# mbrzus/Cross-Modality-Minipig-Gan

Measured on AMD Instinct MI355X. Metric: T1->T2 256x256 slices/sec (G+D step), higher is better.
Workload: dtype f32

## Files before the change

### cross-modality-minipig-gan_amd/csrc/conv_geom.h

```cpp
#pragma once
#include "mpgan_common.h"
#include "norm_fold.h"

namespace mpgan {

typedef float f32x16 __attribute__((ext_vector_type(16)));

constexpr int MAX_PHASES = 27;

struct Phase {
  FastDiv fMx, fMy, fMz;
  int Mz, My, Mx;
  int oz, oy, ox;
  int nz, ny, nx;
  int kz0, ky0, kx0;
  int dz0, dy0, dx0;
};

struct BwdStats {
  const float* z;
  const float* scale;
  const float* shift;
  const float* mean;
  const float* invstd;
// ... 62 lines not shown
    bool found = false;
#pragma unroll
    for (int i = 0; i < MAX_PHASES; ++i) {
      const unsigned tp = i < p.nphase ? (unsigned)(p.tile_start[i + 1] - p.tile_start[i]) : 0u;
      const unsigned lo = (tp * (unsigned)k) >> 3, sz = ((tp * (unsigned)(k + 1)) >> 3) - lo;
      if (!found && r < sz) { ph = i; mt = (int)(lo + r); found = true; }
      if (!found) r -= sz;
    }
    b.phase = ph;
    b.mt = mt;
    b.row = p.tile_start[ph] + mt;
    return b;
  }
  b.nt = (int)(w % (unsigned)p.ntiles);
  unsigned q = w / (unsigned)p.ntiles;
  if (p.phase_outer) {
    b.mt = (int)(q % (unsigned)p.mtiles);
    q /= (unsigned)p.mtiles;
    b.phase = (int)(q % (unsigned)p.nphase);
    b.split = (int)(q / (unsigned)p.nphase);
  } else {
    b.phase = (int)(q % (unsigned)p.nphase);
    q /= (unsigned)p.nphase;
    b.mt = (int)(q % (unsigned)p.mtiles);
    b.split = (int)(q / (unsigned)p.mtiles);
  }
  b.row = b.phase * p.mtiles + b.mt;
  return b;
}
__device__ __forceinline__ BlockId conv_block_id(const GatherConv& p) {
  return decode_block(p, xcd_remap(blockIdx.x, gridDim.x));
// ... 60 lines not shown
      int lo = (g->in_dhw[d] - 1) * g->stride[d] - 2 * g->pad[d] + g->k[d];
      MPGAN_CHECK_ARG(g->out_dhw[d] >= lo && g->out_dhw[d] < lo + g->stride[d],
                      "convT: out_dhw[%d]=%d outside [%d,%d)", d, g->out_dhw[d], lo, lo + g->stride[d]);
    }
  }
  return MPGAN_OK;
}

constexpr int FORM_MIN_BLOCKS_DEFAULT = 1024;
inline void set_geom_flags(GatherConv& p, const mpgan_conv_geom* g) {
  p.mm16 = (g->flags & MPGAN_CONV_MM_BF16) ? 1 : 0;
  p.min_blocks = g->min_blocks > 0 ? g->min_blocks : FORM_MIN_BLOCKS_DEFAULT;
}

bool mm16_gather_ok(const GatherConv& p);
int launch_gather_mm16(const GatherConv& p, int bn, int wraps, int pro, int ks, long maxM, hipStream_t st);

inline void build_forward(GatherConv& p, int n, const int32_t* gath_dhw, int cg, const int32_t* prod_dhw, int cp,
                          const int32_t* k, const int32_t* s, const int32_t* pad) {
  p.N = n; p.Di = gath_dhw[0]; p.Hi = gath_dhw[1]; p.Wi = gath_dhw[2]; p.Cin = cg;
  p.Do = prod_dhw[0]; p.Ho = prod_dhw[1]; p.Wo = prod_dhw[2]; p.Cout = cp;
  p.classes = 0; p.packed = 0;
  p.Kz = k[0]; p.Ky = k[1]; p.Kx = k[2];
  for (int d = 0; d < 3; ++d) { p.ostride[d] = 1; p.istride[d] = s[d]; p.kstep[d] = 1; p.dstep[d] = 1; }
  p.nphase = 1;
  Phase& ph = p.ph[0];
  ph.Mz = prod_dhw[0]; ph.My = prod_dhw[1]; ph.Mx = prod_dhw[2];
  ph.fMx = make_fastdiv(ph.Mx); ph.fMy = make_fastdiv(ph.My); ph.fMz = make_fastdiv(ph.Mz);
  ph.oz = ph.oy = ph.ox = 0;
  ph.nz = k[0]; ph.ny = k[1]; ph.nx = k[2];
  ph.kz0 = ph.ky0 = ph.kx0 = 0;
// ... 104 lines not shown
```

### cross-modality-minipig-gan_amd/csrc/conv_igemm.hip

```cpp
#include "mpgan_common.h"
#include "conv_geom.h"
#include "lds_dma.h"
#include "conv_pipe.h"
#include <stdlib.h>
#include <algorithm>
#include <type_traits>

namespace mpgan {


struct KCursor {
  int ci, jz, jy, jx;
  int delta;
  int dz, dy, dx;
  int woff;
  bool valid;
};

template <int BN, int TM, int TN, int WN, bool SCALAR>
__global__ __launch_bounds__(256) void gather_conv_kernel(const GatherConv p) {
  extern __shared__ __attribute__((aligned(16))) float lds[];
  constexpr int STAGE = (BM + BN) * PITCH;
  constexpr int BROWS = BN / 32;

// ... 1113 lines not shown
  Pipe,
  Dma,
  Kstep,
};

struct GatherChoice {
  GForm form;
  int rc;
  const char* msg;
  int code;
  int rows;
  int arg;
  int pro;
  int bn, wraps, ks;
  bool fast, scalar;
  int cin;
  bool narrow, merge;
  PatchLaunch pl;
  int smem, ntiles, grid;
};
struct BnTile { int bn, tm, tn, wn; };
static BnTile bn_tile(int bn) { return bn == 128 ? BnTile{128, 2, 2, 2} : (bn == 64 ? BnTile{64, 1, 2, 1} : BnTile{32, 1, 1, 1}); }
static bool fuses_bwd_sums(GForm f) { return f == GForm::Mm16 || f == GForm::Pipe || f == GForm::Dma || f == GForm::Kstep; }

template <int CIN, int PRO, bool NARROW, bool MERGE>
__global__ __launch_bounds__(256) void gather_patch_kernel(const GatherConv p, const PatchLaunch pl) {
  extern __shared__ __attribute__((aligned(16))) float lds[];
  typedef float f32x4 __attribute__((ext_vector_type(4)));
  constexpr int PC = CIN + 4;
  constexpr int CQ = CIN / 4;
  constexpr int LU = CIN == 16 ? 3 : (CIN == 32 ? 6 : 12);
  constexpr int WU = CIN == 16 ? 3 : (CIN == 32 ? 9 : 8);
  const int tid = threadIdx.x;
  const int lane = tid & 63, wid = tid >> 6;
  const unsigned wblk = xcd_remap(blockIdx.x, gridDim.x);
  const int phase0 = MERGE ? 0 : (int)(wblk % (unsigned)p.nphase);
  const int nph = MERGE ? p.nphase : 1;
// ... 885 lines not shown


static int select_variant(const GatherConv& p, long maxM, bool thin1, bool thin2) {
  if (thin1) return 1;
  if (thin2) return 2;
  const long mtiles = phase_tile_rows(p, BM);
  static const int force_bn = dev_env("MPGAN_DBG_BN") ? atoi(dev_env("MPGAN_DBG_BN")) : 0;
  if (force_bn == 32 || force_bn == 64 || force_bn == 128) return force_bn;
  int bn = 32;
  if (p.Cout > 64 && mtiles * ((p.Cout + 127) / 128) >= 256) bn = 128;
  else if (p.Cout > 32 && mtiles * ((p.Cout + 63) / 64) >= 256) bn = 64;
  else if (p.Cout > 64 && mtiles * ((p.Cout + 63) / 64) >= 128) bn = 64;
  return bn;
}

template <int BN, int TM, int TN, int WN, int WRAPS, int PRO, bool FAST = false, int KS = 1>
static int launch_pipe_variant(const GatherConv& p, long maxM, hipStream_t st) {
  auto kern = gather_conv_pipe_kernel<BN, TM, TN, WN, WRAPS, PRO, FAST, KS>;
  static const int lds_pad = dev_env("MPGAN_DBG_LDS_PAD") ? atoi(dev_env("MPGAN_DBG_LDS_PAD")) : 0;
  const int smem = KS * 2 * (BM + BN) * PITCH * (int)sizeof(float) + lds_pad;
  if (const int rc = raise_lds_limit<gather_conv_pipe_kernel<BN, TM, TN, WN, WRAPS, PRO, FAST, KS>>(smem, "gather_conv_pipe"))
    return rc;
  GatherConv q = p;
  const long pairs = set_tile_grid(q, BM);
  q.ntiles = (p.Cout + BN - 1) / BN;
  q.phase_outer = (long)p.Cout * p.Cin * p.Kz * p.Ky * p.Kx * 4 > (3L << 20) ? 1 : 0;
  if (q.ksplit < 1) q.ksplit = 1;
  dim3 grid((unsigned)(pairs * q.ntiles * q.ksplit));
  hipLaunchKernelGGL(kern, grid, dim3(256 * KS), smem, st, q);
  return check_launch("gather_conv_pipe");
}

static bool fast_geometry(const GatherConv& p, int bn) {
  static const bool off = dev_env("MPGAN_DBG_NO_FAST") != nullptr;
  if (off || p.nphase != 1 || p.Cout % bn != 0 || p.Cin % 32 != 0 || p.ksplit > 1) return false;
  const Phase& ph = p.ph[0];
  if (ph.nz * ph.ny * ph.nx == 0) return false;
  const int d0[3] = {ph.dz0, ph.dy0, ph.dx0}, nj[3] = {ph.nz, ph.ny, ph.nx}, M[3] = {ph.Mz, ph.My, ph.Mx};
  const int G[3] = {p.Di, p.Hi, p.Wi};
  for (int d = 0; d < 3; ++d) {
    const int lo = p.dstep[d] > 0 ? d0[d] : d0[d] + p.dstep[d] * (nj[d] - 1);
    const int hi = p.dstep[d] > 0 ? d0[d] + p.dstep[d] * (nj[d] - 1) : d0[d];
// ... 1 lines not shown
  }
  return true;
}

static bool pipe_wants_ksplit2(const GatherConv& p, int bn, long maxM) {
  static const bool off = dev_env("MPGAN_DBG_NO_KS2") != nullptr;
  if (off || p.ksplit > 1 || p.Cin % 32 != 0) return false;
  const long blocks = phase_tile_rows(p, BM) * ((p.Cout + bn - 1) / bn);
  if (blocks > 384) return false;
  int min_nk = 1 << 30;
  for (int i = 0; i < p.nphase; ++i) {
    const int nk = p.ph[i].nz * p.ph[i].ny * p.ph[i].nx * p.Cin / BK;
    if (nk > 0 && nk < min_nk) min_nk = nk;
  }
  return min_nk >= 8 && min_nk < (1 << 30);
}

static bool dma_form_ok(const GatherConv& p, int variant, long maxM) {
  static const bool off = dev_env("MPGAN_DBG_NO_DMA") != nullptr;
  if (off || p.pro.scale || p.ksplit > 1 || p.Cin % 32 != 0 || (variant != 128 && variant != 64 && variant != 32)) return false;
  if (p.stats_acc || p.fold.acc) return false;
  const long blocks = phase_tile_rows(p, BM) * ((p.Cout + variant - 1) / variant);
  if (blocks < (p.min_blocks > 0 ? p.min_blocks : FORM_MIN_BLOCKS_DEFAULT)) return false;
  for (int i = 0; i < p.nphase; ++i) {
    const int nt = p.ph[i].nz * p.ph[i].ny * p.ph[i].nx;
    if (nt < 1 || nt > 32) return false;
  }
  const long bytes_a = (long)p.N * p.Di * p.Hi * p.Wi * p.ldi * 4, ktot4 = (long)p.Kz * p.Ky * p.Kx * p.Cin * 4;
  return bytes_a < (long)HW_OOB && (long)p.Cout * ktot4 < (long)HW_OOB && ktot4 < 0xFFFF;
}
// ... 6 lines not shown
  if (const int rc = raise_lds_limit<gather_conv_dma_kernel<BN, TM, TN, WN, NST>>(smem, "gather_conv_dma")) return rc;
  GatherConv q = p;
  const long pairs = set_tile_grid(q, BM);
  q.ntiles = (p.Cout + BN - 1) / BN;
  q.phase_outer = (long)p.Cout * p.Cin * p.Kz * p.Ky * p.Kx * 4 > (3L << 20) ? 1 : 0;
  q.ksplit = 1;
  dim3 grid((unsigned)(pairs * q.ntiles));
  hipLaunchKernelGGL(kern, grid, dim3(256), smem, st, q);
  return check_launch("gather_conv_dma");
}

template <int WRAPS, int PRO>
static int launch_pipe_bn(const GatherConv& p, const GatherChoice& c, long maxM, hipStream_t st) {
  if constexpr (WRAPS == 1 && PRO == 3) {
    if (c.fast) return launch_pipe_variant<128, 2, 2, 2, 1, 3, true>(p, maxM, st);
  }
  if constexpr (WRAPS == 1 && PRO != 3) {
    if (c.ks == 2) {
      if (c.bn == 64) return launch_pipe_variant<64, 1, 2, 1, 1, PRO, false, 2>(p, maxM, st);
      return launch_pipe_variant<32, 1, 1, 1, 1, PRO, false, 2>(p, maxM, st);
    }
  }
  if (c.bn == 128) return launch_pipe_variant<128, 2, 2, 2, WRAPS, PRO>(p, maxM, st);
  if (c.bn == 64) return launch_pipe_variant<64, 1, 2, 1, WRAPS, PRO>(p, maxM, st);
  return launch_pipe_variant<32, 1, 1, 1, WRAPS, PRO>(p, maxM, st);
}

template <int WRAPS>
static int launch_pipe_pro(const GatherConv& p, const GatherChoice& c, long maxM, hipStream_t st) {
  switch (c.pro) {
// ... 389 lines not shown
      c.narrow = p.Cout <= 16;
      c.merge = c.pl.merged != 0;
      c.form = persist ? GForm::PatchPersist : GForm::Patch;
      if (persist) {
        c.pl = pp;
        c.smem = psmem;
      }
      return c;
    }
    CHOICE_REFUSE(p.stats != nullptr, "gather_conv: fused statistics of a patch-kernel geometry need 16-byte "
                                      "aligned operands (the partial-row count differs otherwise)");
  }
  CHOICE_REFUSE(p.fold.acc != nullptr, "gather_conv: fold-on-load is served by the persistent patch kernel only");
  c.rows = (int)phase_tile_rows(p, BM);
  c.ks = 1;
  const bool vec = (p.Cin % 4 == 0) && (p.ldi % 4 == 0) && ((reinterpret_cast<uintptr_t>(p.in) & 15) == 0) &&
                   ((reinterpret_cast<uintptr_t>(p.wp) & 15) == 0) &&
                   (!p.pro.scale || (((reinterpret_cast<uintptr_t>(p.pro.scale) |
                                       reinterpret_cast<uintptr_t>(p.pro.shift)) & 15) == 0 &&
                                     p.pro.n_stride % 4 == 0));
  static const bool no_pipe = dev_env("MPGAN_DBG_NO_PIPE") != nullptr;
  const bool small = (long)p.N * p.Di * p.Hi * p.Wi * p.ldi * 4 < (1L << 32) &&
                     (long)p.Cout * p.Cin * p.Kz * p.Ky * p.Kx * 4 < (1L << 32) &&
                     (long)p.N * (p.pro.n_stride > 0 ? p.pro.n_stride : 0) * 4 < (1L << 31);
  const bool mm16 = p.mm16 && vec && small && mm16_gather_ok(p);
  if (vec && small && (p.Cin % 32 == 0 || p.Cin == 16) && (!no_pipe || mm16)) {
    c.form = GForm::Pipe;
    c.wraps = p.Cin % 32 == 0 ? 1 : 2;
    if (!p.pro.scale) c.pro = 0;
    else if (p.pro.n_stride == 0 && p.pro.act == MPGAN_ACT_LEAKY && !p.pro.slope_ptr && p.pro.slope >= 0.f && p.pro.slope <= 1.f)
      c.pro = 3;
    else c.pro = p.pro.n_stride == 0 ? 1 : 2;
    const bool ks2 = c.wraps == 1 && variant != 128 && pipe_wants_ksplit2(p, variant, maxM);
    if (c.wraps == 1 && c.pro == 3 && variant == 128 && fast_geometry(p, 128)) {
      c.fast = true;
      c.code = 1128;
    } else if (c.wraps == 1 && c.pro != 3 && ks2) {
      c.ks = 2;
      c.code = 2000 + variant;
    } else if (c.wraps == 1 && c.pro == 0 && dma_form_ok(p, variant, maxM)) {
      c.form = GForm::Dma;
      c.code = 3000 + variant;
    }
    if (mm16) {
      c.form = GForm::Mm16;
      c.pro = p.pro.scale != nullptr;
      c.ks = ks2 ? 2 : 1;
      c.fast = false;
    }
    return c;
  }
  c.form = GForm::Kstep;
  c.scalar = !vec;
  return c;
}
#undef CHOICE_REFUSE

static int launch_chosen(const GatherConv& p, const GatherChoice& c, long maxM, hipStream_t st) {
  if (c.rc != MPGAN_OK) {
    set_error("%s", c.msg);
    return c.rc;
  }
// ... 83 lines not shown
    case GForm::Patch3d:
      if (c.arg) return c.pro ? launch_patch3d_instance<true, true>(p, st) : launch_patch3d_instance<false, true>(p, st);
      return c.pro ? launch_patch3d_instance<true, false>(p, st) : launch_patch3d_instance<false, false>(p, st);
    case GForm::Patch: return launch_patch<false>(p, c, c.pl, st);
    case GForm::PatchPersist: {
      static void* zp = nullptr;
      if (!zp && hipGetSymbolAddress(&zp, HIP_SYMBOL(g_patch_zero_page)) != hipSuccess) {
        zp = nullptr;
        set_error("gather_patch_persist: no address for the zero page");
        return MPGAN_ERR_HIP;
      }
      PatchLaunch pl = c.pl;
      pl.zero_page = zp;
      return launch_patch<true>(p, c, pl, st);
    }
    case GForm::Mm16: return launch_gather_mm16(p, c.bn, c.wraps, c.pro, c.ks, maxM, st);
    case GForm::Pipe: return c.wraps == 1 ? launch_pipe_pro<1>(p, c, maxM, st) : launch_pipe_pro<2>(p, c, maxM, st);
    case GForm::Dma:
      if (c.bn == 128) return launch_dma_variant<128, 2, 2, 2>(p, maxM, st);
      if (c.bn == 64) return launch_dma_variant<64, 1, 2, 1>(p, maxM, st);
      return launch_dma_variant<32, 1, 1, 1, 2>(p, maxM, st);
    case GForm::Kstep:
      if (c.scalar) {
        if (c.bn == 128) return launch_variant<128, 2, 2, 2, true>(p, maxM, st);
        if (c.bn == 64) return launch_variant<64, 1, 2, 1, true>(p, maxM, st);
        return launch_variant<32, 1, 1, 1, true>(p, maxM, st);
      }
      if (c.bn == 128) return launch_variant<128, 2, 2, 2, false>(p, maxM, st);
      if (c.bn == 64) return launch_variant<64, 1, 2, 1, false>(p, maxM, st);
      return launch_variant<32, 1, 1, 1, false>(p, maxM, st);
  }
  return MPGAN_ERR_UNSUPPORTED;
}

static int gather_kernel_name(const GatherChoice& c, char* buf, int len) {
  const char* b[2] = {"false", "true"};
  const BnTile t = bn_tile(c.bn);
  switch (c.form) {
    case GForm::ThinBf16OutRows: return snprintf(buf, len, "thin_cin1_rows_kernel<%d, true>", c.arg);
    case GForm::Cin1Rows: return snprintf(buf, len, "thin_cin1_rows_kernel<%d, false>", c.arg);
    case GForm::ThinBf16OutFull: return snprintf(buf, len, "thin_cin1_full_kernel<%d, true>", c.arg);
    case GForm::Cin1Full: return snprintf(buf, len, "thin_cin1_full_kernel<%d, false>", c.arg);
    case GForm::ThinBf16InMfma: return snprintf(buf, len, "thin_cout1_mfma_bf16_kernel");
    case GForm::ThinBf16In: return snprintf(buf, len, "thin_cout1_kernel<%d, true>", c.arg);
    case GForm::C1C1Rows4: return snprintf(buf, len, "thin_c1c1_rows4_kernel<%s>", b[c.arg]);
    case GForm::Cin1: return snprintf(buf, len, "thin_cin1_kernel<%d>", c.arg);
    case GForm::ConvtQuad: return snprintf(buf, len, "convt_quad_cout1_kernel<%d>", c.arg);
    case GForm::ConvtOct: return snprintf(buf, len, "convt_oct_cout1_kernel<%d>", c.arg);
    case GForm::Cout1: return snprintf(buf, len, "thin_cout1_kernel<%d, false>", c.arg);
    case GForm::Patch3d: return snprintf(buf, len, "gather_patch3d_c16_kernel<%s, %s>", b[c.pro], b[c.arg]);
    case GForm::Patch:
      return snprintf(buf, len, "gather_patch_kernel<%d, %d, %s, %s>", c.cin, c.pro, b[c.narrow], b[c.merge]);
// ... 338 lines not shown
```

### cross-modality-minipig-gan_amd/csrc/conv_mm16.hip

```cpp
#include "conv_pipe.h"
#include "wgrad_pipe.h"
#include <stdlib.h>

namespace mpgan {

template <int BN, int TM, int TN, int WN, int WRAPS, int PRO, int KS>
static int launch_mm16_variant(const GatherConv& p, long maxM, hipStream_t st) {
  auto kern = gather_conv_pipe_kernel<BN, TM, TN, WN, WRAPS, PRO, false, KS, true>;
  constexpr int stage_b = (BM + BN) * MM16_PITCHB;
  constexpr int loop_b = KS * 2 * stage_b;
  constexpr int fold_b = KS > 1 ? TM * TN * 16 * 256 * 4 : 0;
  constexpr int epi_b = CONV_EPI_FLOATS * 4;
  constexpr int smem = loop_b > fold_b ? (loop_b > epi_b ? loop_b : epi_b) : (fold_b > epi_b ? fold_b : epi_b);
  if (const int rc = raise_lds_limit<gather_conv_pipe_kernel<BN, TM, TN, WN, WRAPS, PRO, false, KS, true>>(
          smem, "gather_conv_pipe (bf16 operands)"))
    return rc;
  GatherConv q = p;
  const long pairs = set_tile_grid(q, BM);
  q.ntiles = (p.Cout + BN - 1) / BN;
  q.phase_outer = (long)p.Cout * p.Cin * p.Kz * p.Ky * p.Kx * 4 > (3L << 20) ? 1 : 0;
  q.ksplit = 1;
  dim3 grid((unsigned)(pairs * q.ntiles));
  hipLaunchKernelGGL(kern, grid, dim3(256 * KS), smem, st, q);
  return check_launch("gather_conv_pipe (bf16 operands)");
}

template <int WRAPS, int PRO>
static int launch_mm16_bn(const GatherConv& p, int bn, int ks, long maxM, hipStream_t st) {
  if constexpr (WRAPS == 1) {
    if (ks == 2)
      return bn == 64 ? launch_mm16_variant<64, 1, 2, 1, 1, PRO, 2>(p, maxM, st)
                      : launch_mm16_variant<32, 1, 1, 1, 1, PRO, 2>(p, maxM, st);
  }
  if (bn == 128) return launch_mm16_variant<128, 2, 2, 2, WRAPS, PRO, 1>(p, maxM, st);
  if (bn == 64) return launch_mm16_variant<64, 1, 2, 1, WRAPS, PRO, 1>(p, maxM, st);
  return launch_mm16_variant<32, 1, 1, 1, WRAPS, PRO, 1>(p, maxM, st);
}

bool mm16_gather_ok(const GatherConv& p) {
  static const bool off = dev_env("MPGAN_DBG_NO_MM16") != nullptr;
  return !off && (p.Cin % 32 == 0 || p.Cin == 16) && (!p.pro.scale || p.pro.n_stride == 0) && !p.fold.acc &&
         !p.stats_acc && p.ksplit <= 1 && !p.in_bf16 && !p.out_bf16;
}

int launch_gather_mm16(const GatherConv& p, int bn, int wraps, int pro, int ks, long maxM, hipStream_t st) {
  if (wraps == 1) return pro ? launch_mm16_bn<1, 1>(p, bn, ks, maxM, st) : launch_mm16_bn<1, 0>(p, bn, ks, maxM, st);
  return pro ? launch_mm16_bn<2, 1>(p, bn, ks, maxM, st) : launch_mm16_bn<2, 0>(p, bn, ks, maxM, st);
}

template <int BD, int BG, int TM, int TN, int WN, int PRO, bool PAD>
static int launch_wgrad_mm16_variant(const WgradParams& p, hipStream_t st) {
  auto kern = wgrad_pipe_kernel<BD, BG, TM, TN, WN, PRO, PAD, true>;
  constexpr int smem = 2 * WBK * (BD + BG) * (int)sizeof(float) + 2 * 32 * 16;
  if (const int rc = raise_lds_limit<wgrad_pipe_kernel<BD, BG, TM, TN, WN, PRO, PAD, true>>(smem, "wgrad_pipe (bf16 operands)"))
    return rc;
  dim3 grid((unsigned)p.tiles_c * p.tiles_d * p.nsplit);
  hipLaunchKernelGGL(kern, grid, dim3(256), smem, st, p);
  return check_launch("wgrad_pipe (bf16 operands)");
}

template <int PRO>
static int launch_wgrad_mm16_pad(const WgradParams& p, int BD, int BG, hipStream_t st) {
// ... 16 lines not shown
```

### cross-modality-minipig-gan_amd/csrc/conv_pipe.h

```cpp
#pragma once
#include <type_traits>
#include "mpgan_common.h"
#include "conv_geom.h"
#include "lds_dma.h"

namespace mpgan {

constexpr int BM = 128;
constexpr int BK = 32;
constexpr int PITCH = BK + 4;

#ifndef MPGAN_BWD_EPILOGUE_WALK
#define MPGAN_BWD_EPILOGUE_WALK 0
#endif

__device__ __forceinline__ void bwd_sums_add(float v, float zz, float sc, float sh, float mu, float is, bool leaky, float slope,
                                             float& b1, float& b2, float& b3) {
#pragma clang fp contract(off)
  const float y = __builtin_fmaf(zz, sc, sh);
  const float zh = (zz - mu) * is;
  const bool neg = leaky && y < 0.f;
  const float gy = neg ? v * slope : v;
  const float t3 = neg ? v * y : 0.f;
  b1 += gy;
  b2 = __builtin_fmaf(gy, zh, b2);
  b3 += t3;
}

template <int BN, int TM, int TN, int WN, bool BWC = false>
__device__ __forceinline__ void conv_epilogue(const GatherConv& p, const Phase& ph, f32x16 (&acc)[TM][TN], float* lds,
                                              long m0, int n0, long Mtot, int stats_row, bool zero_rows = false,
                                              int tid = threadIdx.x, bool active = true, const float* bias_pre = nullptr) {
  const int lane = tid & 63, wid = tid >> 6;
  const int li = lane & 31, lh = lane >> 5;
  const int wm = wid / WN, wn = wid % WN;
  const int Cout = p.Cout;
  const int ksplit_id = p.ksplit > 1 ? (int)(xcd_remap(blockIdx.x, gridDim.x) / (unsigned)(p.ntiles * p.mtiles * (p.packed ? 1 : p.nphase))) : 0;
  int* rowpix = reinterpret_cast<int*>(lds);
  const bool bw = p.bwd.part != nullptr;
  int* rowoo = rowpix + BM;
  int* rowoz = rowpix + 2 * BM;
  bool bw_vec = false;
  if constexpr (BWC) if (bw) {
    const unsigned long long npix = (unsigned long long)p.N * p.Do * p.Ho * p.Wo;
    bw_vec = !MPGAN_BWD_EPILOGUE_WALK && !p.epi.scale && !p.resid && !p.tanh_out && (Cout % 4 == 0) && (p.ldo % 4 == 0) &&
             ((reinterpret_cast<uintptr_t>(p.out) & 15) == 0) && Cout <= p.ldo && Cout <= p.bwd.ldz &&
             npix * (unsigned)p.ldo * 4ull <= 0xFFFFFFFFull && npix * (unsigned)p.bwd.ldz * 4ull <= 0xFFFFFFFFull;
  }
  if (active && tid < BM) {
    const unsigned m = (unsigned)m0 + tid;
    int pix = -1;
    if (m < (unsigned)Mtot) {
      unsigned q, umx, umy, umz;
      fdivmod(m, ph.fMx, q, umx);
      fdivmod(q, ph.fMy, q, umy);
      fdivmod(q, ph.fMz, q, umz);
      const int mx = (int)umx, my = (int)umy, mz = (int)umz;
      const int n = (int)q;
      int oz = mz * p.ostride[0] + ph.oz, oy = my * p.ostride[1] + ph.oy, ox = mx * p.ostride[2] + ph.ox;
      if (oz < p.Do && oy < p.Ho && ox < p.Wo) pix = ((n * p.Do + oz) * p.Ho + oy) * p.Wo + ox;
    }
    rowpix[tid] = pix;
    if (bw_vec) {
      const unsigned upix = pix < 0 ? 0u : (unsigned)pix;
// ... 231 lines not shown
    constexpr int WM = 4 / WN;
    float* st = lds + 1024;
    int* nvp = reinterpret_cast<int*>(lds) + 512;
    if (zero_rows && active) {
#pragma unroll
      for (int tm = 0; tm < TM; ++tm)
#pragma unroll
        for (int r = 0; r < 16; ++r) {
          const int row = (wm * TM + tm) * 32 + (r & 3) + 8 * (r >> 2) + 4 * lh;
          if (rowpix[row] < 0) {
#pragma unroll
            for (int tn = 0; tn < TN; ++tn) acc[tm][tn][r] = 0.f;
          }
        }
    }
    if (active && tid < BM) {
      const unsigned long long b = __ballot(rowpix[tid] >= 0);
      if (lane == 0) nvp[wid] = __popcll(b);
    }
#pragma unroll
    for (int tn = 0; tn < TN; ++tn) {
      const int col = (wn * TN + tn) * 32 + li;
      float sm = 0.f, sq = 0.f;
#pragma unroll
      for (int tm = 0; tm < TM; ++tm)
#pragma unroll
        for (int r = 0; r < 16; ++r) {
          const float v = acc[tm][tn][r];
          sm += v;
          sq = fmaf(v, v, sq);
        }
      sm += __shfl_xor(sm, 32, 64);
      sq += __shfl_xor(sq, 32, 64);
      if (active && lh == 0) {
        st[(wm * 2 + 0) * BN + col] = sm;
        st[(wm * 2 + 1) * BN + col] = sq;
      }
    }
    __syncthreads();
    if (active && tid < BN && n0 + tid < Cout) {
      float sm = 0.f, sq = 0.f;
#pragma unroll
      for (int w = 0; w < WM; ++w) {
        sm += st[(w * 2 + 0) * BN + tid];
        sq += st[(w * 2 + 1) * BN + tid];
      }
      const float nv = (float)(nvp[0] + nvp[1]);
      const float b = p.bias ? p.bias[n0 + tid] : 0.f;
      if (p.stats_acc) {
        long long* rep = p.stats_acc + (long)(blockIdx.x % (unsigned)p.acc_rep) * ACC_WORDS * Cout;
        acc_add(rep, Cout, 0, n0 + tid, sm + nv * b);
        acc_add(rep, Cout, 2, n0 + tid, sq + b * (2.f * sm + nv * b));
      } else {
      float* row = p.stats + (long)stats_row * 2 * Cout;
      row[n0 + tid] = sm + nv * b;
      row[Cout + n0 + tid] = sq + b * (2.f * sm + nv * b);
      }
    }
  }
}

typedef __bf16 mm_bf16x8 __attribute__((ext_vector_type(8)));
typedef __bf16 mm_bf16x4 __attribute__((ext_vector_type(4)));
constexpr int MM16_PITCHB = 80;
constexpr int CONV_EPI_FLOATS = 2048 + 4 * 32 * 36 + 1024;

template <int BN, int TM, int TN, int WN, int WRAPS, int PRO, bool FAST = false, int KS = 1, bool MM16 = false>
__global__ __launch_bounds__(256 * KS) void gather_conv_pipe_kernel(const GatherConv p) {
  extern __shared__ __attribute__((aligned(16))) float lds_all[];
  constexpr int STAGE = MM16 ? (BM + BN) * (MM16_PITCHB / 4) : (BM + BN) * PITCH;
  constexpr int BROWS = BN / 32;
  constexpr int NMF = 4 * TM * TN;

  const int tid = threadIdx.x & 255;
  const int kg = KS > 1 ? (int)(threadIdx.x >> 8) : 0;
  float* lds = lds_all + kg * 2 * STAGE;
  const int lane = tid & 63, wid = tid >> 6;
  const int li = lane & 31, lh = lane >> 5;
  const int wm = wid / WN, wn = wid % WN;
  MPGAN_STAMP(p, 0);
  MPGAN_STAMP_VALUE(p, 6, 1);
  const BlockId bid = conv_block_id(p);
  const Phase ph = p.ph[bid.phase];
  const long Mtot = (long)p.N * ph.Mz * ph.My * ph.Mx;
  const long m0 = (long)bid.mt * BM;
  const int n0 = bid.nt * BN;
  const int stats_row = bid.row;
  if (m0 >= Mtot) {
    if (p.stats && kg == 0 && tid < BN && n0 + tid < p.Cout) {
      float* row = p.stats + (long)stats_row * 2 * p.Cout;
      row[n0 + tid] = 0.f;
      row[p.Cout + n0 + tid] = 0.f;
    }
    if (p.bwd.part && kg == 0 && tid < BN && n0 + tid < p.Cout) {
      float* row = p.bwd.part + (long)stats_row * 3 * p.Cout;
      row[n0 + tid] = 0.f;
      row[p.Cout + n0 + tid] = 0.f;
      row[2 * p.Cout + n0 + tid] = 0.f;
    }
    return;
// ... 2 lines not shown
  const int ntaps = ph.nz * ph.ny * ph.nx;
  const int Kp = ntaps * Cin;
  const int nk_all = (Kp + BK - 1) / BK;
  const int nk_per = (nk_all + p.ksplit * KS - 1) / (p.ksplit * KS);
  const int kt_begin = (bid.split * KS + kg) * nk_per;
  const int nk = nk_all - kt_begin < nk_per ? (nk_all - kt_begin > 0 ? nk_all - kt_begin : 0) : nk_per;
  const long Ktot = (long)p.Kz * p.Ky * p.Kx * Cin;
  const float* __restrict__ gin = p.in;
  const float* __restrict__ gw = p.wp;
  const float* __restrict__ gscale = p.pro.scale;
  const float* __restrict__ gshift = p.pro.shift;
  const int nstride = p.pro.n_stride, act = p.pro.act;
  const float slope = PRO ? pro_slope(p.pro) : 1.f;

  const int cc = tid & 7, r0 = tid >> 3;
  int rn[4], rz[4], ry[4], rx[4];
  unsigned rbB[4];
#pragma unroll
  for (int i = 0; i < 4; ++i) {
    unsigned m = (unsigned)m0 + r0 + 32 * i;
    if constexpr (FAST) m = m < (unsigned)Mtot ? m : (unsigned)Mtot - 1u;
    if (m < (unsigned)Mtot) {
      unsigned q, umx, umy, umz;
      fdivmod(m, ph.fMx, q, umx);
      fdivmod(q, ph.fMy, q, umy);
      fdivmod(q, ph.fMz, q, umz);
      const int mx = (int)umx, my = (int)umy, mz = (int)umz;
      rn[i] = (int)q;
      rz[i] = mz * p.istride[0];
      ry[i] = my * p.istride[1];
      rx[i] = mx * p.istride[2];
    } else {
      rn[i] = 0;
      rz[i] = ry[i] = rx[i] = -(1 << 28);
// ... 74 lines not shown
      ci += BK / WRAPS;
      const int wc = ci >= Cin ? 1 : 0;
      ci -= (-wc) & Cin;
      jx += wc;
      const int wx = jx == ph.nx ? 1 : 0;
      jx -= (-wx) & ph.nx;
      jy += wx;
      const int wy = jy == ph.ny ? 1 : 0;
      jy -= (-wy) & ph.ny;
      jz += wy;
    }
    place();
  };

  struct Stage {
    float4 ra[4], rb[BROWS], rsc[PRO == 2 ? 4 : 1], rsh[PRO == 2 ? 4 : 1];
    unsigned amask;
    int kvalid;
  };
  Stage SX, SY;

  auto issue_loads = [&](Stage& S) {
    float4 (&ra)[4] = S.ra;
    float4 (&rb)[BROWS] = S.rb;
    auto& rsc = S.rsc;
    auto& rsh = S.rsh;
    unsigned amask = 0;
    S.kvalid = cmask;
    const int tci = UCUR ? ci + 4 * cc : ci;
    const unsigned cisB = (unsigned)(tci & cmask) * 4u;
#pragma unroll
    for (int i = 0; i < 4; ++i) {
      int ok = cmask;
      if constexpr (!FAST) {
        const int iz = rz[i] + dz, iy = ry[i] + dy, ix = rx[i] + dx;
        ok = ((unsigned)iz < (unsigned)Di ? cmask : 0) & ((unsigned)iy < (unsigned)Hi ? -1 : 0) &
             ((unsigned)ix < (unsigned)Wi ? -1 : 0);
      }
      const unsigned boff = (rbB[i] + deltaB + (unsigned)tci * 4u) & (unsigned)ok;
      ra[i] = *reinterpret_cast<const float4*>(ginb + boff);
      if constexpr (!FAST) amask |= ((unsigned)ok & 1u) << i;
      if constexpr (PRO == 2) {
        const unsigned sb = (unsigned)(rn[i] * nstride) * 4u + cisB;
        rsc[i] = *reinterpret_cast<const float4*>(gscb + sb);
        rsh[i] = *reinterpret_cast<const float4*>(gshb + sb);
      }
    }
    if constexpr (PRO == 1 || PRO == 3) {
      rsc[0] = *reinterpret_cast<const float4*>(gscb + cisB);
      rsh[0] = *reinterpret_cast<const float4*>(gshb + cisB);
    }
    const unsigned wkB = (unsigned)(woff + tci) * 4u;
#pragma unroll
    for (int i = 0; i < BROWS; ++i)
      rb[i] = *reinterpret_cast<const float4*>(gwb + ((wrowB[i] + wkB) & (unsigned)cmask));
    S.amask = amask;
    advance();
  };

  auto store_tile = [&](int buf, const Stage& S) {
    const float4 (&ra)[4] = S.ra;
    const float4 (&rb)[BROWS] = S.rb;
    const auto& rsc = S.rsc;
    const auto& rsh = S.rsh;
    const unsigned amask = S.amask;
    const int kvalid = S.kvalid;
    float* As = lds + buf * STAGE;
    float* Bs = As + (MM16 ? BM * (MM16_PITCHB / 4) : BM * PITCH);
#pragma unroll
    for (int i = 0; i < 4; ++i) {
      float4 v = ra[i];
      if constexpr (PRO == 3) {
        const float4 sc = rsc[0], sh = rsh[0];
        v.x = v.x * sc.x + sh.x; v.y = v.y * sc.y + sh.y; v.z = v.z * sc.z + sh.z; v.w = v.w * sc.w + sh.w;
        v.x = fmaxf(v.x, v.x * slope); v.y = fmaxf(v.y, v.y * slope);
        v.z = fmaxf(v.z, v.z * slope); v.w = fmaxf(v.w, v.w * slope);
      } else if constexpr (PRO != 0) {
        const float4 sc = rsc[PRO == 2 ? i : 0], sh = rsh[PRO == 2 ? i : 0];
        v.x = act_apply(v.x * sc.x + sh.x, act, slope);
        v.y = act_apply(v.y * sc.y + sh.y, act, slope);
        v.z = act_apply(v.z * sc.z + sh.z, act, slope);
        v.w = act_apply(v.w * sc.w + sh.w, act, slope);
      }
      if constexpr (!FAST) {
        const bool ok = (amask >> i) & 1u;
// ... 37 lines not shown
    const int co = n0 + (wn * TN + tn) * 32 + li;
    bias_pre[tn] = (p.bias && co < Cout) ? p.bias[co] : 0.f;
  }

  if (nk > 0) {
    issue_loads(SY);
    issue_loads(SX);
    store_tile(0, SY);
  }
  __syncthreads();
  MPGAN_STAMP(p, 1);

  auto step = [&](int cb, Stage& Sn, const Stage& Sp) {
    if constexpr (MM16) {
      const char* Ab = reinterpret_cast<const char*>(lds + cb * STAGE) + (wm * TM * 32 + li) * MM16_PITCHB + 16 * lh;
      const char* Bb = reinterpret_cast<const char*>(lds + cb * STAGE) + (BM + wn * TN * 32 + li) * MM16_PITCHB + 16 * lh;
      mm_bf16x8 a[2][TM], b[2][TN];
#pragma unroll
      for (int s = 0; s < 2; ++s) {
#pragma unroll
        for (int tm = 0; tm < TM; ++tm) a[s][tm] = *reinterpret_cast<const mm_bf16x8*>(Ab + tm * 32 * MM16_PITCHB + 32 * s);
#pragma unroll
        for (int tn = 0; tn < TN; ++tn) b[s][tn] = *reinterpret_cast<const mm_bf16x8*>(Bb + tn * 32 * MM16_PITCHB + 32 * s);
      }
      issue_loads(Sn);
#pragma unroll
      for (int tm = 0; tm < TM; ++tm)
#pragma unroll
        for (int tn = 0; tn < TN; ++tn)
          acc[tm][tn] = __builtin_amdgcn_mfma_f32_32x32x16_bf16(a[0][tm], b[0][tn], acc[tm][tn], 0, 0, 0);
      store_tile(cb ^ 1, Sp);
#pragma unroll
      for (int tm = 0; tm < TM; ++tm)
#pragma unroll
        for (int tn = 0; tn < TN; ++tn)
          acc[tm][tn] = __builtin_amdgcn_mfma_f32_32x32x16_bf16(a[1][tm], b[1][tn], acc[tm][tn], 0, 0, 0);
      return;
    }
    const float* As = lds + cb * STAGE + (wm * TM * 32 + li) * PITCH + 4 * lh;
    const float* Bs = lds + cb * STAGE + BM * PITCH + (wn * TN * 32 + li) * PITCH + 4 * lh;
    float4 a[2][TM], b[2][TN];
    auto read_group = [&](int g, int slot) {
#pragma unroll
      for (int tm = 0; tm < TM; ++tm)
        a[slot][tm] = *reinterpret_cast<const float4*>(As + tm * 32 * PITCH + 8 * g);
#pragma unroll
      for (int tn = 0; tn < TN; ++tn)
        b[slot][tn] = *reinterpret_cast<const float4*>(Bs + tn * 32 * PITCH + 8 * g);
    };
    read_group(0, 0);
    __builtin_amdgcn_sched_barrier(0);
#pragma unroll
    for (int g = 0; g < 4; ++g) {
      const int sl = g & 1;
      if (g < 3) read_group(g + 1, sl ^ 1);
// ... 29 lines not shown
      __builtin_amdgcn_sched_barrier(0);
    }
  };

  if constexpr (KS == 1) {
    for (int kt = 0; kt < nk; kt += 2) {
      step(0, SY, SX);
      __syncthreads();
      if (kt + 1 < nk) {
        step(1, SX, SY);
        __syncthreads();
      }
    }
    MPGAN_STAMP(p, 2);
    MPGAN_STAMP(p, 3);
    conv_epilogue<BN, TM, TN, WN>(p, ph, acc, lds, m0, n0, Mtot, stats_row, FAST && m0 + BM > Mtot, threadIdx.x, true, bias_pre);
    MPGAN_STAMP(p, 7);
  } else {
    for (int kt = 0; kt < nk_per; kt += 2) {
      if (kt < nk) step(0, SY, SX);
      __syncthreads();
      if (kt + 1 < nk_per) {
        if (kt + 1 < nk) step(1, SX, SY);
        __syncthreads();
      }
    }
    MPGAN_STAMP(p, 2);
    float* red = lds_all;
    for (int g = 1; g < KS; ++g) {
      if (kg == g) {
#pragma unroll
// ... 3 lines not shown
#pragma unroll
            for (int r = 0; r < 16; ++r) red[((a * TN + b) * 16 + r) * 256 + tid] = acc[a][b][r];
      }
      __syncthreads();
      if (kg == 0) {
#pragma unroll
        for (int a = 0; a < TM; ++a)
#pragma unroll
          for (int b = 0; b < TN; ++b)
#pragma unroll
            for (int r = 0; r < 16; ++r) acc[a][b][r] += red[((a * TN + b) * 16 + r) * 256 + tid];
      }
      __syncthreads();
    }
    MPGAN_STAMP(p, 3);
    conv_epilogue<BN, TM, TN, WN>(p, ph, acc, lds_all, m0, n0, Mtot, stats_row, FAST && m0 + BM > Mtot, tid, kg == 0, bias_pre);
    MPGAN_STAMP(p, 7);
  }
}

}
```

Before: 301.9.

## Add half-height M tiles with K-split and interleaved phase ordering for small grids

Adds a half-height (64-row) tile variant of the pipelined gather conv kernel, with BN=64 and K-split 2. It is chosen for flat 2D geometries that would otherwise use BN=32 with K-split, so B operand reuse improves while the block count stays up. It also adds a phase ordering for small grids with unequal per-phase tap counts that interleaves heavy and light transposed-conv phases across neighbouring blocks, to balance load. In exchange it adds more kernel instantiations, parameterises the epilogue row count, and refuses the path in some fused-statistics cases.

```diff
diff --git a/cross-modality-minipig-gan_amd/csrc/conv_geom.h b/cross-modality-minipig-gan_amd/csrc/conv_geom.h
--- a/cross-modality-minipig-gan_amd/csrc/conv_geom.h
+++ b/cross-modality-minipig-gan_amd/csrc/conv_geom.h
@@ -100,7 +100,15 @@
   }
   b.nt = (int)(w % (unsigned)p.ntiles);
   unsigned q = w / (unsigned)p.ntiles;
-  if (p.phase_outer) {
+  if (p.phase_outer == 2) {
+    const unsigned slot = q % (unsigned)p.nphase;
+    q /= (unsigned)p.nphase;
+    b.mt = (int)(q % (unsigned)p.mtiles);
+    b.split = (int)(q / (unsigned)p.mtiles);
+    const int a = (slot & 1u) ? (int)(slot >> 1) : p.nphase - 1 - (int)(slot >> 1);
+    const bool mirror = ((q * (unsigned)(p.nphase * p.ntiles)) >> 5) & 1u;
+    b.phase = mirror ? p.nphase - 1 - a : a;
+  } else if (p.phase_outer) {
     b.mt = (int)(q % (unsigned)p.mtiles);
     q /= (unsigned)p.mtiles;
     b.phase = (int)(q % (unsigned)p.nphase);
@@ -191,7 +199,7 @@
 }
 
 bool mm16_gather_ok(const GatherConv& p);
-int launch_gather_mm16(const GatherConv& p, int bn, int wraps, int pro, int ks, long maxM, hipStream_t st);
+int launch_gather_mm16(const GatherConv& p, int bn, int wraps, int pro, int ks, bool half, long maxM, hipStream_t st);
 
 inline void build_forward(GatherConv& p, int n, const int32_t* gath_dhw, int cg, const int32_t* prod_dhw, int cp,
                           const int32_t* k, const int32_t* s, const int32_t* pad) {
diff --git a/cross-modality-minipig-gan_amd/csrc/conv_igemm.hip b/cross-modality-minipig-gan_amd/csrc/conv_igemm.hip
--- a/cross-modality-minipig-gan_amd/csrc/conv_igemm.hip
+++ b/cross-modality-minipig-gan_amd/csrc/conv_igemm.hip
@@ -1151,13 +1151,17 @@
   int pro;
   int bn, wraps, ks;
   bool fast, scalar;
+  bool half;
   int cin;
   bool narrow, merge;
   PatchLaunch pl;
   int smem, ntiles, grid;
 };
 struct BnTile { int bn, tm, tn, wn; };
-static BnTile bn_tile(int bn) { return bn == 128 ? BnTile{128, 2, 2, 2} : (bn == 64 ? BnTile{64, 1, 2, 1} : BnTile{32, 1, 1, 1}); }
+static BnTile bn_tile(int bn, bool half = false) {
+  if (half) return BnTile{64, 1, 1, 2};
+  return bn == 128 ? BnTile{128, 2, 2, 2} : (bn == 64 ? BnTile{64, 1, 2, 1} : BnTile{32, 1, 1, 1});
+}
 static bool fuses_bwd_sums(GForm f) { return f == GForm::Mm16 || f == GForm::Pipe || f == GForm::Dma || f == GForm::Kstep; }
 
 template <int CIN, int PRO, bool NARROW, bool MERGE>
@@ -2073,18 +2077,29 @@
   return bn;
 }
 
+static bool phases_unequal(const GatherConv& p) {
+  const int t0 = p.ph[0].nz * p.ph[0].ny * p.ph[0].nx;
+  for (int i = 1; i < p.nphase; ++i)
+    if (p.ph[i].nz * p.ph[i].ny * p.ph[i].nx != t0) return true;
+  return false;
+}
+
 template <int BN, int TM, int TN, int WN, int WRAPS, int PRO, bool FAST = false, int KS = 1>
 static int launch_pipe_variant(const GatherConv& p, long maxM, hipStream_t st) {
   auto kern = gather_conv_pipe_kernel<BN, TM, TN, WN, WRAPS, PRO, FAST, KS>;
+  constexpr int BMT = (4 / WN) * TM * 32;
   static const int lds_pad = dev_env("MPGAN_DBG_LDS_PAD") ? atoi(dev_env("MPGAN_DBG_LDS_PAD")) : 0;
-  const int smem = KS * 2 * (BM + BN) * PITCH * (int)sizeof(float) + lds_pad;
+  const int smem = KS * 2 * (BMT + BN) * PITCH * (int)sizeof(float) + lds_pad;
+  static_assert(KS * 2 * (BMT + BN) * PITCH >= CONV_EPI_FLOATS || KS == 1, "the fold and the epilogue use the K groups' stages");
   if (const int rc = raise_lds_limit<gather_conv_pipe_kernel<BN, TM, TN, WN, WRAPS, PRO, FAST, KS>>(smem, "gather_conv_pipe"))
     return rc;
   GatherConv q = p;
-  const long pairs = set_tile_grid(q, BM);
+  const long pairs = set_tile_grid(q, BMT);
   q.ntiles = (p.Cout + BN - 1) / BN;
   q.phase_outer = (long)p.Cout * p.Cin * p.Kz * p.Ky * p.Kx * 4 > (3L << 20) ? 1 : 0;
   if (q.ksplit < 1) q.ksplit = 1;
+  static const bool no_mix = dev_env("MPGAN_DBG_NO_PHASE_MIX") != nullptr;
+  if (!no_mix && !q.phase_outer && !q.packed && q.nphase > 1 && pairs * q.ntiles * q.ksplit <= 512 && phases_unequal(q)) q.phase_outer = 2;
   dim3 grid((unsigned)(pairs * q.ntiles * q.ksplit));
   hipLaunchKernelGGL(kern, grid, dim3(256 * KS), smem, st, q);
   return check_launch("gather_conv_pipe");
@@ -2116,6 +2131,12 @@
     if (nk > 0 && nk < min_nk) min_nk = nk;
   }
   return min_nk >= 8 && min_nk < (1 << 30);
+}
+
+static bool pipe_wants_half(const GatherConv& p, int bn, long maxM) {
+  static const bool off = dev_env("MPGAN_DBG_NO_HALF") != nullptr;
+  const bool flat = p.Kz == 1 && p.Di == 1 && p.Do == 1;
+  return !off && flat && bn == 32 && p.Cout > 32 && pipe_wants_ksplit2(p, bn, maxM);
 }
 
 static bool dma_form_ok(const GatherConv& p, int variant, long maxM) {
@@ -2152,6 +2173,9 @@
 static int launch_pipe_bn(const GatherConv& p, const GatherChoice& c, long maxM, hipStream_t st) {
   if constexpr (WRAPS == 1 && PRO == 3) {
     if (c.fast) return launch_pipe_variant<128, 2, 2, 2, 1, 3, true>(p, maxM, st);
+  }
+  if constexpr (WRAPS == 1) {
+    if (c.half) return launch_pipe_variant<64, 1, 1, 2, 1, PRO, false, 2>(p, maxM, st);
   }
   if constexpr (WRAPS == 1 && PRO != 3) {
     if (c.ks == 2) {
@@ -2571,6 +2595,7 @@
   CHOICE_REFUSE(p.fold.acc != nullptr, "gather_conv: fold-on-load is served by the persistent patch kernel only");
   c.rows = (int)phase_tile_rows(p, BM);
   c.ks = 1;
+  const bool half = p.Cin % 32 == 0 && pipe_wants_half(p, variant, maxM);
   const bool vec = (p.Cin % 4 == 0) && (p.ldi % 4 == 0) && ((reinterpret_cast<uintptr_t>(p.in) & 15) == 0) &&
                    ((reinterpret_cast<uintptr_t>(p.wp) & 15) == 0) &&
                    (!p.pro.scale || (((reinterpret_cast<uintptr_t>(p.pro.scale) |
@@ -2581,6 +2606,9 @@
                      (long)p.Cout * p.Cin * p.Kz * p.Ky * p.Kx * 4 < (1L << 32) &&
                      (long)p.N * (p.pro.n_stride > 0 ? p.pro.n_stride : 0) * 4 < (1L << 31);
   const bool mm16 = p.mm16 && vec && small && mm16_gather_ok(p);
+  CHOICE_REFUSE(half && !(vec && small && (!no_pipe || mm16)) && (p.stats || p.bwd.part),
+                "gather_conv: fused statistics / norm-backward sums of a half-height-tile geometry need 16-byte aligned "
+                "operands below 4 GiB (the partial-row count differs otherwise)");
   if (vec && small && (p.Cin % 32 == 0 || p.Cin == 16) && (!no_pipe || mm16)) {
     c.form = GForm::Pipe;
     c.wraps = p.Cin % 32 == 0 ? 1 : 2;
@@ -2589,7 +2617,13 @@
       c.pro = 3;
     else c.pro = p.pro.n_stride == 0 ? 1 : 2;
     const bool ks2 = c.wraps == 1 && variant != 128 && pipe_wants_ksplit2(p, variant, maxM);
-    if (c.wraps == 1 && c.pro == 3 && variant == 128 && fast_geometry(p, 128)) {
+    if (half) {
+      c.half = true;
+      c.ks = 2;
+      c.bn = 64;
+      c.code = 2064;
+      c.rows = (int)phase_tile_rows(p, BM / 2);
+    } else if (c.wraps == 1 && c.pro == 3 && variant == 128 && fast_geometry(p, 128)) {
       c.fast = true;
       c.code = 1128;
     } else if (c.wraps == 1 && c.pro != 3 && ks2) {
@@ -2602,7 +2636,7 @@
     if (mm16) {
       c.form = GForm::Mm16;
       c.pro = p.pro.scale != nullptr;
-      c.ks = ks2 ? 2 : 1;
+      c.ks = (ks2 || half) ? 2 : 1;
       c.fast = false;
     }
     return c;
@@ -2716,7 +2750,7 @@
       pl.zero_page = zp;
       return launch_patch<true>(p, c, pl, st);
     }
-    case GForm::Mm16: return launch_gather_mm16(p, c.bn, c.wraps, c.pro, c.ks, maxM, st);
+    case GForm::Mm16: return launch_gather_mm16(p, c.bn, c.wraps, c.pro, c.ks, c.half, maxM, st);
     case GForm::Pipe: return c.wraps == 1 ? launch_pipe_pro<1>(p, c, maxM, st) : launch_pipe_pro<2>(p, c, maxM, st);
     case GForm::Dma:
       if (c.bn == 128) return launch_dma_variant<128, 2, 2, 2>(p, maxM, st);
@@ -2737,7 +2771,7 @@
 
 static int gather_kernel_name(const GatherChoice& c, char* buf, int len) {
   const char* b[2] = {"false", "true"};
-  const BnTile t = bn_tile(c.bn);
+  const BnTile t = bn_tile(c.bn, (c.form == GForm::Pipe || c.form == GForm::Mm16) && c.half);
   switch (c.form) {
     case GForm::ThinBf16OutRows: return snprintf(buf, len, "thin_cin1_rows_kernel<%d, true>", c.arg);
     case GForm::Cin1Rows: return snprintf(buf, len, "thin_cin1_rows_kernel<%d, false>", c.arg);
diff --git a/cross-modality-minipig-gan_amd/csrc/conv_mm16.hip b/cross-modality-minipig-gan_amd/csrc/conv_mm16.hip
--- a/cross-modality-minipig-gan_amd/csrc/conv_mm16.hip
+++ b/cross-modality-minipig-gan_amd/csrc/conv_mm16.hip
@@ -7,7 +7,8 @@
 template <int BN, int TM, int TN, int WN, int WRAPS, int PRO, int KS>
 static int launch_mm16_variant(const GatherConv& p, long maxM, hipStream_t st) {
   auto kern = gather_conv_pipe_kernel<BN, TM, TN, WN, WRAPS, PRO, false, KS, true>;
-  constexpr int stage_b = (BM + BN) * MM16_PITCHB;
+  constexpr int BMT = (4 / WN) * TM * 32;
+  constexpr int stage_b = (BMT + BN) * MM16_PITCHB;
   constexpr int loop_b = KS * 2 * stage_b;
   constexpr int fold_b = KS > 1 ? TM * TN * 16 * 256 * 4 : 0;
   constexpr int epi_b = CONV_EPI_FLOATS * 4;
@@ -16,7 +17,7 @@
           smem, "gather_conv_pipe (bf16 operands)"))
     return rc;
   GatherConv q = p;
-  const long pairs = set_tile_grid(q, BM);
+  const long pairs = set_tile_grid(q, BMT);
   q.ntiles = (p.Cout + BN - 1) / BN;
   q.phase_outer = (long)p.Cout * p.Cin * p.Kz * p.Ky * p.Kx * 4 > (3L << 20) ? 1 : 0;
   q.ksplit = 1;
@@ -26,8 +27,9 @@
 }
 
 template <int WRAPS, int PRO>
-static int launch_mm16_bn(const GatherConv& p, int bn, int ks, long maxM, hipStream_t st) {
+static int launch_mm16_bn(const GatherConv& p, int bn, int ks, bool half, long maxM, hipStream_t st) {
   if constexpr (WRAPS == 1) {
+    if (half) return launch_mm16_variant<64, 1, 1, 2, 1, PRO, 2>(p, maxM, st);
     if (ks == 2)
       return bn == 64 ? launch_mm16_variant<64, 1, 2, 1, 1, PRO, 2>(p, maxM, st)
                       : launch_mm16_variant<32, 1, 1, 1, 1, PRO, 2>(p, maxM, st);
@@ -43,9 +45,9 @@
          !p.stats_acc && p.ksplit <= 1 && !p.in_bf16 && !p.out_bf16;
 }
 
-int launch_gather_mm16(const GatherConv& p, int bn, int wraps, int pro, int ks, long maxM, hipStream_t st) {
-  if (wraps == 1) return pro ? launch_mm16_bn<1, 1>(p, bn, ks, maxM, st) : launch_mm16_bn<1, 0>(p, bn, ks, maxM, st);
-  return pro ? launch_mm16_bn<2, 1>(p, bn, ks, maxM, st) : launch_mm16_bn<2, 0>(p, bn, ks, maxM, st);
+int launch_gather_mm16(const GatherConv& p, int bn, int wraps, int pro, int ks, bool half, long maxM, hipStream_t st) {
+  if (wraps == 1) return pro ? launch_mm16_bn<1, 1>(p, bn, ks, half, maxM, st) : launch_mm16_bn<1, 0>(p, bn, ks, half, maxM, st);
+  return pro ? launch_mm16_bn<2, 1>(p, bn, ks, false, maxM, st) : launch_mm16_bn<2, 0>(p, bn, ks, false, maxM, st);
 }
 
 template <int BD, int BG, int TM, int TN, int WN, int PRO, bool PAD>
diff --git a/cross-modality-minipig-gan_amd/csrc/conv_pipe.h b/cross-modality-minipig-gan_amd/csrc/conv_pipe.h
--- a/cross-modality-minipig-gan_amd/csrc/conv_pipe.h
+++ b/cross-modality-minipig-gan_amd/csrc/conv_pipe.h
@@ -27,7 +27,7 @@
   b3 += t3;
 }
 
-template <int BN, int TM, int TN, int WN, bool BWC = false>
+template <int BN, int TM, int TN, int WN, bool BWC = false, int BMT = BM>
 __device__ __forceinline__ void conv_epilogue(const GatherConv& p, const Phase& ph, f32x16 (&acc)[TM][TN], float* lds,
                                               long m0, int n0, long Mtot, int stats_row, bool zero_rows = false,
                                               int tid = threadIdx.x, bool active = true, const float* bias_pre = nullptr) {
@@ -38,8 +38,9 @@
   const int ksplit_id = p.ksplit > 1 ? (int)(xcd_remap(blockIdx.x, gridDim.x) / (unsigned)(p.ntiles * p.mtiles * (p.packed ? 1 : p.nphase))) : 0;
   int* rowpix = reinterpret_cast<int*>(lds);
   const bool bw = p.bwd.part != nullptr;
-  int* rowoo = rowpix + BM;
-  int* rowoz = rowpix + 2 * BM;
+  static_assert(BMT == BM || (BMT == BM / 2 && !BWC), "conv_epilogue: full- or half-height tiles; path C is full-height");
+  int* rowoo = rowpix + BMT;
+  int* rowoz = rowpix + 2 * BMT;
   bool bw_vec = false;
   if constexpr (BWC) if (bw) {
     const unsigned long long npix = (unsigned long long)p.N * p.Do * p.Ho * p.Wo;
@@ -47,7 +48,7 @@
              ((reinterpret_cast<uintptr_t>(p.out) & 15) == 0) && Cout <= p.ldo && Cout <= p.bwd.ldz &&
              npix * (unsigned)p.ldo * 4ull <= 0xFFFFFFFFull && npix * (unsigned)p.bwd.ldz * 4ull <= 0xFFFFFFFFull;
   }
-  if (active && tid < BM) {
+  if (active && tid < BMT) {
     const unsigned m = (unsigned)m0 + tid;
     int pix = -1;
     if (m < (unsigned)Mtot) {
@@ -309,7 +310,7 @@
           }
         }
     }
-    if (active && tid < BM) {
+    if (active && tid < BMT) {
       const unsigned long long b = __ballot(rowpix[tid] >= 0);
       if (lane == 0) nvp[wid] = __popcll(b);
     }
@@ -340,7 +341,7 @@
         sm += st[(w * 2 + 0) * BN + tid];
         sq += st[(w * 2 + 1) * BN + tid];
       }
-      const float nv = (float)(nvp[0] + nvp[1]);
+      const float nv = (float)(BMT > 64 ? nvp[0] + nvp[1] : nvp[0]);
       const float b = p.bias ? p.bias[n0 + tid] : 0.f;
       if (p.stats_acc) {
         long long* rep = p.stats_acc + (long)(blockIdx.x % (unsigned)p.acc_rep) * ACC_WORDS * Cout;
@@ -363,7 +364,10 @@
 template <int BN, int TM, int TN, int WN, int WRAPS, int PRO, bool FAST = false, int KS = 1, bool MM16 = false>
 __global__ __launch_bounds__(256 * KS) void gather_conv_pipe_kernel(const GatherConv p) {
   extern __shared__ __attribute__((aligned(16))) float lds_all[];
-  constexpr int STAGE = MM16 ? (BM + BN) * (MM16_PITCHB / 4) : (BM + BN) * PITCH;
+  constexpr int BMT = (4 / WN) * TM * 32;
+  constexpr int AR = BMT / 32;
+  static_assert(BMT == BM || BMT == BM / 2, "gather_conv_pipe_kernel: full- or half-height tiles");
+  constexpr int STAGE = MM16 ? (BMT + BN) * (MM16_PITCHB / 4) : (BMT + BN) * PITCH;
   constexpr int BROWS = BN / 32;
   constexpr int NMF = 4 * TM * TN;
 
@@ -378,7 +382,7 @@
   const BlockId bid = conv_block_id(p);
   const Phase ph = p.ph[bid.phase];
   const long Mtot = (long)p.N * ph.Mz * ph.My * ph.Mx;
-  const long m0 = (long)bid.mt * BM;
+  const long m0 = (long)bid.mt * BMT;
   const int n0 = bid.nt * BN;
   const int stats_row = bid.row;
   if (m0 >= Mtot) {
@@ -411,10 +415,10 @@
   const float slope = PRO ? pro_slope(p.pro) : 1.f;
 
   const int cc = tid & 7, r0 = tid >> 3;
-  int rn[4], rz[4], ry[4], rx[4];
-  unsigned rbB[4];
-#pragma unroll
-  for (int i = 0; i < 4; ++i) {
+  int rn[AR], rz[AR], ry[AR], rx[AR];
+  unsigned rbB[AR];
+#pragma unroll
+  for (int i = 0; i < AR; ++i) {
     unsigned m = (unsigned)m0 + r0 + 32 * i;
     if constexpr (FAST) m = m < (unsigned)Mtot ? m : (unsigned)Mtot - 1u;
     if (m < (unsigned)Mtot) {
@@ -519,14 +523,14 @@
   };
 
   struct Stage {
-    float4 ra[4], rb[BROWS], rsc[PRO == 2 ? 4 : 1], rsh[PRO == 2 ? 4 : 1];
+    float4 ra[AR], rb[BROWS], rsc[PRO == 2 ? AR : 1], rsh[PRO == 2 ? AR : 1];
     unsigned amask;
     int kvalid;
   };
   Stage SX, SY;
 
   auto issue_loads = [&](Stage& S) {
-    float4 (&ra)[4] = S.ra;
+    float4 (&ra)[AR] = S.ra;
     float4 (&rb)[BROWS] = S.rb;
     auto& rsc = S.rsc;
     auto& rsh = S.rsh;
@@ -535,7 +539,7 @@
     const int tci = UCUR ? ci + 4 * cc : ci;
     const unsigned cisB = (unsigned)(tci & cmask) * 4u;
 #pragma unroll
-    for (int i = 0; i < 4; ++i) {
+    for (int i = 0; i < AR; ++i) {
       int ok = cmask;
       if constexpr (!FAST) {
         const int iz = rz[i] + dz, iy = ry[i] + dy, ix = rx[i] + dx;
@@ -564,16 +568,16 @@
   };
 
   auto store_tile = [&](int buf, const Stage& S) {
-    const float4 (&ra)[4] = S.ra;
+    const float4 (&ra)[AR] = S.ra;
     const float4 (&rb)[BROWS] = S.rb;
     const auto& rsc = S.rsc;
     const auto& rsh = S.rsh;
     const unsigned amask = S.amask;
     const int kvalid = S.kvalid;
     float* As = lds + buf * STAGE;
-    float* Bs = As + (MM16 ? BM * (MM16_PITCHB / 4) : BM * PITCH);
-#pragma unroll
-    for (int i = 0; i < 4; ++i) {
+    float* Bs = As + (MM16 ? BMT * (MM16_PITCHB / 4) : BMT * PITCH);
+#pragma unroll
+    for (int i = 0; i < AR; ++i) {
       float4 v = ra[i];
       if constexpr (PRO == 3) {
         const float4 sc = rsc[0], sh = rsh[0];
@@ -641,7 +645,7 @@
   auto step = [&](int cb, Stage& Sn, const Stage& Sp) {
     if constexpr (MM16) {
       const char* Ab = reinterpret_cast<const char*>(lds + cb * STAGE) + (wm * TM * 32 + li) * MM16_PITCHB + 16 * lh;
-      const char* Bb = reinterpret_cast<const char*>(lds + cb * STAGE) + (BM + wn * TN * 32 + li) * MM16_PITCHB + 16 * lh;
+      const char* Bb = reinterpret_cast<const char*>(lds + cb * STAGE) + (BMT + wn * TN * 32 + li) * MM16_PITCHB + 16 * lh;
       mm_bf16x8 a[2][TM], b[2][TN];
 #pragma unroll
       for (int s = 0; s < 2; ++s) {
@@ -665,7 +669,7 @@
       return;
     }
     const float* As = lds + cb * STAGE + (wm * TM * 32 + li) * PITCH + 4 * lh;
-    const float* Bs = lds + cb * STAGE + BM * PITCH + (wn * TN * 32 + li) * PITCH + 4 * lh;
+    const float* Bs = lds + cb * STAGE + BMT * PITCH + (wn * TN * 32 + li) * PITCH + 4 * lh;
     float4 a[2][TM], b[2][TN];
     auto read_group = [&](int g, int slot) {
 #pragma unroll
@@ -725,7 +729,7 @@
     }
     MPGAN_STAMP(p, 2);
     MPGAN_STAMP(p, 3);
-    conv_epilogue<BN, TM, TN, WN>(p, ph, acc, lds, m0, n0, Mtot, stats_row, FAST && m0 + BM > Mtot, threadIdx.x, true, bias_pre);
+    conv_epilogue<BN, TM, TN, WN, false, BMT>(p, ph, acc, lds, m0, n0, Mtot, stats_row, FAST && m0 + BMT > Mtot, threadIdx.x, true, bias_pre);
     MPGAN_STAMP(p, 7);
   } else {
     for (int kt = 0; kt < nk_per; kt += 2) {
@@ -759,7 +763,7 @@
       __syncthreads();
     }
     MPGAN_STAMP(p, 3);
-    conv_epilogue<BN, TM, TN, WN>(p, ph, acc, lds_all, m0, n0, Mtot, stats_row, FAST && m0 + BM > Mtot, tid, kg == 0, bias_pre);
+    conv_epilogue<BN, TM, TN, WN, false, BMT>(p, ph, acc, lds_all, m0, n0, Mtot, stats_row, FAST && m0 + BMT > Mtot, tid, kg == 0, bias_pre);
     MPGAN_STAMP(p, 7);
   }
 }
```

Result: no change. 302.2, median of 6 (+0.1%).
